# JiaoXianjun/multi-rtl-sdr-calibration

Hardware: AMD Instinct MI355X
Metric: IQ Msamples/s through FCCH+SCH calib (higher is better)
Workload: dtype f64; 1 GPU; cfg4 full chain gsm_sync_demod.m:107-124: 64 dongle streams (64/GPU) x 1020000 IQ samples (102 frames), fir1(46), FCCH+SCH+total_ppm_calculation, table on the host; streams_per_gpu=64, streams_total=64, output=table, collective=none, rows_checked_vs_oracle_per_rank=0

## Files before the change

### include/gsmcal.h

```cpp
#ifndef GSMCAL_H
#define GSMCAL_H

#include <stddef.h>
#include <stdint.h>

#ifdef __cplusplus
extern "C" {
#endif

typedef struct gsmcal_ctx gsmcal_ctx;

enum {
    GSMCAL_OK = 0,
    GSMCAL_S_NO_FCCH = 1,
    GSMCAL_S_FEW_HITS = 2,
    GSMCAL_S_FINE_FEW = 3,
    GSMCAL_S_FINE_SPACING = 4,
    GSMCAL_S_FINE_FEW_BURSTS = 5,
    GSMCAL_S_FINE_LOW_SNR = 6,
    GSMCAL_S_SCH_EDGE = 7,
    GSMCAL_S_SCH_FEW = 8,
    GSMCAL_S_SCH_SPACING = 9,
    GSMCAL_S_POST_NO_POS = 10,
    GSMCAL_S_POST_FEW_BCCH = 11,
// ... 247 lines not shown
int gsmcal_allgather_table(gsmcal_ctx* ctx, gsmcal_comm* comm, const double* d_local, int rows_per_rank, int cols,
                           double* d_all);

int gsmcal_allgather_table_async(gsmcal_ctx* ctx, gsmcal_comm* comm, const double* d_local, int rows_per_rank, int cols,
                                 double* d_all, int slot);
int gsmcal_allgather_wait(gsmcal_ctx* ctx, int slot);
int gsmcal_allgather_sync(gsmcal_ctx* ctx, int slot);

typedef struct gsmcal_ring gsmcal_ring;
int gsmcal_ring_create(gsmcal_ctx* ctx, size_t batch_bytes, int slots, gsmcal_ring** out);
void gsmcal_ring_destroy(gsmcal_ring* ring);
void* gsmcal_ring_host(gsmcal_ring* ring, int slot);
int gsmcal_ring_submit(gsmcal_ring* ring, int slot, size_t bytes);
void* gsmcal_ring_acquire(gsmcal_ring* ring, int slot);
int gsmcal_ring_release(gsmcal_ring* ring, int slot);
int gsmcal_ring_host_ready(gsmcal_ring* ring, int slot);

int gsmcal_synth_expand_dev(gsmcal_ctx* ctx, const uint8_t* d_base, int k, long n, uint8_t* d_out, long d,
                            long first_unit, unsigned long long seed);

int gsmcal_last_batch_details(gsmcal_ctx* ctx, int d, double* coarse_pos, double* coarse_snr,
                              double* fine_first, double* fcch_pos, double* sch_first, int* counts);

int gsmcal_last_batch_snr(gsmcal_ctx* ctx, int stream, double* snr, long cap, long* n_table, long* n_moving);

#ifdef __cplusplus
}
#endif
#endif
```

### multi-rtl-sdr-calibration_amd/__init__.py

```python
from . import build, ingest, synth
from ._lib import GsmcalError, MAX_HITS, MAX_POS_ROWS, MAX_SUBBANDS, TABLE_COLS, DEMOD_COLS, MAX_BCCH, BCCH_COLS, SCH_COLS, HYPERFRAME, CW_MAX_EVENTS, CW_COLS, CW_TILE, CW_OK, CW_SHORT, CW_ZERO, SIGNATURES, lib_path, load
from .api import (
    Context, default_context, raw2iq, filter, chn_filter_8x_4x, chn_filter_4x, move_fft_snr_runtime_avg,
    specific_fft_snr_fix_avg, FCCH_coarse_position, FCCH_fine_correction, SCH_corr_rate_correction,
    carrier_correct_post_SCH, total_ppm_calculation, SCH_equalise, frontend_batch, fcch_scan_batch, calibrate_batch,
    last_batch_details, last_batch_snr, TABLE_FIELDS, fcch_scan_batch_dev, calibrate_batch_dev, synth_expand_dev,
    set_verbose, last_call_report, num2str, band_power_batch, band_power_batch_dev, split_spectrum_scan,
    diversity_spectrum_scan, FCCH_demod, fcch_demod_batch, fcch_demod_batch_dev, demod_rows, DEMOD_FIELDS,
    subband_power_batch, subband_power_batch_dev, multichannel_spectrum_scan, CW_check, cw_check_batch, cw_check_batch_dev,
    cw_rows, CW_FIELDS, BCCH_demod, bcch_demod_batch, bcch_demod_batch_dev, bcch_rows, BCCH_FIELDS,
    SCH_decode, sch_decode_batch, sch_decode_batch_dev, sch_rows, SCH_FIELDS, sch_alignment,
)
```

### multi-rtl-sdr-calibration_amd/_lib.py

```python
from __future__ import annotations

import ctypes as C
import os

from . import build as _build

_LIB = None

c_double_p = C.POINTER(C.c_double)
c_int_p = C.POINTER(C.c_int)
c_long_p = C.POINTER(C.c_long)
c_u8_p = C.POINTER(C.c_uint8)

MAX_HITS = 24
MAX_POS_ROWS = 6 * MAX_HITS
TABLE_COLS = 10
MAX_SUBBANDS = 16
CW_MAX_EVENTS = 16
CW_COLS = 5 + 2 * CW_MAX_EVENTS
CW_TILE = 2048
CW_OK, CW_SHORT, CW_ZERO = 0, 1, 2
DEMOD_COLS = 4 + 3 * MAX_HITS
MAX_BCCH = 4 * MAX_HITS
BCCH_COLS = 6 + 4 * MAX_BCCH
# ... 95 lines not shown
    "gsmcal_comm_init_file": (C.c_int, [C.c_void_p, C.c_char_p, C.c_int, C.c_int, C.POINTER(C.c_void_p)]),
    "gsmcal_last_batch_snr": (C.c_int, [C.c_void_p, C.c_int, c_double_p, C.c_long, c_long_p, c_long_p]),
    "gsmcal_comm_init_file_nonce": (C.c_int, [C.c_void_p, C.c_char_p, C.c_ulonglong, C.c_int, C.c_int, C.POINTER(C.c_void_p)]),
    "gsmcal_comm_default_nonce": (C.c_ulonglong, []),
    "gsmcal_comm_id_file_exchange": (C.c_int, [C.c_char_p, C.c_ulonglong, C.c_int, C.c_int, C.c_void_p, C.c_double]),
    "gsmcal_comm_id_file_exchange_aged": (C.c_int, [C.c_char_p, C.c_ulonglong, C.c_int, C.c_int, C.c_void_p, C.c_double]),
    "gsmcal_comm_id_file_remove": (C.c_int, [C.c_char_p]),
    "gsmcal_comm_destroy": (None, [C.c_void_p]),
    "gsmcal_allgather_table": (C.c_int, [C.c_void_p, C.c_void_p, C.c_void_p, C.c_int, C.c_int, C.c_void_p]),
    "gsmcal_allgather_table_async": (C.c_int, [C.c_void_p, C.c_void_p, C.c_void_p, C.c_int, C.c_int, C.c_void_p, C.c_int]),
    "gsmcal_allgather_wait": (C.c_int, [C.c_void_p, C.c_int]),
    "gsmcal_allgather_sync": (C.c_int, [C.c_void_p, C.c_int]),
    "gsmcal_ring_create": (C.c_int, [C.c_void_p, C.c_size_t, C.c_int, C.POINTER(C.c_void_p)]),
    "gsmcal_ring_destroy": (None, [C.c_void_p]),
    "gsmcal_ring_host": (C.c_void_p, [C.c_void_p, C.c_int]),
    "gsmcal_ring_submit": (C.c_int, [C.c_void_p, C.c_int, C.c_size_t]),
    "gsmcal_ring_acquire": (C.c_void_p, [C.c_void_p, C.c_int]),
    "gsmcal_ring_release": (C.c_int, [C.c_void_p, C.c_int]),
    "gsmcal_ring_host_ready": (C.c_int, [C.c_void_p, C.c_int]),
    "gsmcal_synth_expand_dev": (C.c_int, [C.c_void_p, C.c_void_p, C.c_int, C.c_long, C.c_void_p, C.c_long, C.c_long,
                                          C.c_ulonglong]),
    "gsmcal_last_batch_details": (C.c_int, [C.c_void_p, C.c_int, c_double_p, c_double_p, c_double_p, c_double_p,
                                            c_double_p, c_int_p]),
}


class Params(C.Structure):
    _fields_ = [("coarse_th_db", C.c_double), ("coarse_mv_factor", C.c_int), ("coarse_max_offset", C.c_int),
                ("min_hits", C.c_int), ("fine_max_offset", C.c_int), ("fine_max_ppm", C.c_double),
                ("fine_gate_snr_db", C.c_double), ("fine_noise_bw_hz", C.c_double), ("sch_max_offset", C.c_int),
                ("sch_max_ppm", C.c_double), ("post_min_bcch", C.c_int), ("scan_min_hits", C.c_int),
                ("scan_spacing", C.c_double), ("scan_spacing_idle", C.c_double), ("scan_tol", C.c_double)]


SIGNATURES.update({
    "gsmcal_params_default": (None, [C.POINTER(Params)]),
    "gsmcal_set_params": (C.c_int, [C.c_void_p, C.POINTER(Params)]),
    "gsmcal_get_params": (C.c_int, [C.c_void_p, C.POINTER(Params)]),
})


class GsmcalError(RuntimeError):
    pass


def lib_path():
# ... 43 lines not shown
```

### multi-rtl-sdr-calibration_amd/api.py

```python
from __future__ import annotations

import ctypes as C
import math
import os

import numpy as np

from . import _lib
from ._lib import BCCH_COLS, SCH_COLS, CW_COLS, CW_MAX_EVENTS, DEMOD_COLS, MAX_BCCH, MAX_HITS, MAX_POS_ROWS, TABLE_COLS, GsmcalError

_CTX = {}


_VERBOSE = [os.environ.get("GSMCAL_VERBOSE") == "1"]


def set_verbose(on=True):
    _VERBOSE[0] = bool(on)


def last_call_report(ctx=None):
    ctx = ctx or default_context()
    n = ctx.lib.gsmcal_last_call_report(ctx.h, None, 0)
    if n <= 0:
# ... 775 lines not shown
    ctx = ctx or default_context()
    coef = np.ascontiguousarray(coef, dtype=np.float64)
    vp = lambda p: C.c_void_p(p) if p else None
    ctx.check(ctx.lib.gsmcal_fcch_scan_batch_dev(ctx.h, C.c_void_p(d_raw), int(d), int(n), _dp(coef), len(coef),
                                                 C.c_void_p(d_snr_numhit), vp(d_positions), vp(d_pos_snr), vp(d_counts)),
              "fcch_scan_batch_dev")


def synth_expand_dev(d_base, k, n, d_out, d, first_unit=0, seed=20260101, ctx=None):
    ctx = ctx or default_context()
    ctx.check(ctx.lib.gsmcal_synth_expand_dev(ctx.h, C.c_void_p(d_base), int(k), int(n), C.c_void_p(d_out), int(d),
                                              int(first_unit), int(seed)), "synth_expand_dev")


def last_batch_snr(stream, ctx=None):
    ctx = ctx or default_context()
    buf = np.zeros(1 << 16)
    n_tab, n_mov = C.c_long(0), C.c_long(0)
    ctx.check(ctx.lib.gsmcal_last_batch_snr(ctx.h, int(stream), _dp(buf), len(buf), C.byref(n_tab), C.byref(n_mov)),
              "last_batch_snr")
    return buf[: min(n_tab.value, len(buf))].copy(), int(n_mov.value)


def last_batch_details(d, ctx=None):
    ctx = ctx or default_context()
    arrs = [np.zeros((d, MAX_HITS)) for _ in range(5)]
    counts = np.zeros((d, 5), dtype=np.int32)
    ctx.check(ctx.lib.gsmcal_last_batch_details(ctx.h, d, *[_dp(a) for a in arrs],
                                                counts.ctypes.data_as(_lib.c_int_p)), "last_batch_details")
    names = ("coarse_pos", "coarse_snr", "fine_first", "fcch_pos", "sch_first")
    out = {k: a for k, a in zip(names, arrs)}
    out["counts"] = counts
    return out
```

### multi-rtl-sdr-calibration_amd/csrc/abi_calls.h

```cpp
#pragma once

const char* gsmcal_version(void) { return GSMCAL_VERSION; }

void gsmcal_params_default(gsmcal_params* p) {
    if (!p) return;
    p->coarse_th_db = 10.0; p->coarse_mv_factor = 10; p->coarse_max_offset = 5; p->min_hits = 5;
    p->fine_max_offset = 64; p->fine_max_ppm = 4000.0; p->fine_gate_snr_db = 5.0; p->fine_noise_bw_hz = 200e3;
    p->sch_max_offset = 8; p->sch_max_ppm = 400.0; p->post_min_bcch = 4;
    p->scan_min_hits = 3; p->scan_spacing = 12500.0; p->scan_spacing_idle = 12500.0 + 1250.0; p->scan_tol = 50.0;
}

int gsmcal_set_params(gsmcal_ctx* c, const gsmcal_params* p) {
    if (!c || !p) return GSMCAL_E_ARG;
    RET_IF(pipe_join(c));
    gsmcal_params d;
    gsmcal_params_default(&d);
    if (p->coarse_mv_factor != d.coarse_mv_factor || p->coarse_max_offset != d.coarse_max_offset ||
        p->fine_max_offset != d.fine_max_offset || p->fine_noise_bw_hz != d.fine_noise_bw_hz || p->sch_max_offset != d.sch_max_offset) {
        c->err = "gsmcal_set_params: a geometry field differs from its default";
        return GSMCAL_E_UNSUPPORTED;
    }
    if (p->min_hits < 2 || p->min_hits > GSMCAL_MAX_HITS || p->scan_min_hits < 1 || p->post_min_bcch < 0) {
        c->err = "gsmcal_set_params: min_hits outside 2..GSMCAL_MAX_HITS, scan_min_hits < 1 or post_min_bcch < 0";
        return GSMCAL_E_ARG;
// ... 54 lines not shown
    gsmcal_ctx* c = new gsmcal_ctx();
    gsmcal_params_default(&c->params);
    c->device = device_id;
    c->stream = (hipStream_t)hip_stream;
    c->own_stream = false;
    c->lanes[0].stream = c->stream;
    c->cur = &c->lanes[0];
    const char* e = getenv("GSMCAL_LANES");
    if (e && atoi(e) >= 1) c->n_lanes_cfg = atoi(e) > MAX_LANES ? MAX_LANES : atoi(e);
    { int ncu = 0; if (hipDeviceGetAttribute(&ncu, hipDeviceAttributeMultiprocessorCount, c->device) == hipSuccess && ncu > 0) c->n_cu = ncu; }
    { int lds = 0; if (hipDeviceGetAttribute(&lds, hipDeviceAttributeMaxSharedMemoryPerMultiprocessor, c->device) == hipSuccess && lds > 0) c->lds_per_cu = (size_t)lds; }
    if (const char* e2 = getenv("GSMCAL_SNR_INLINE_MIN")) c->snr_inline_min = atoi(e2);
    if (const char* e2 = getenv("GSMCAL_SNR_INLINE_KEEP")) c->snr_inline_keep = atoi(e2);
    if (const char* e2 = getenv("GSMCAL_FRONT_NT")) c->front_nt = atoi(e2);
    if (const char* e2 = getenv("GSMCAL_SCAN_SPLIT")) c->scan_split = atoi(e2);
    const char* sst = getenv("GSMCAL_SCAN_STAGES");
    if (sst && atoi(sst) >= 1) c->scan_stages = atoi(sst);
    const char* lm = getenv("GSMCAL_LANE_MIN");
    if (lm && atoi(lm) >= 1) c->lane_min = atoi(lm);
    const char* ce = getenv("GSMCAL_CERT");
    if (ce) c->certify = atoi(ce) != 0;
    const char* sfe = getenv("GSMCAL_SNR_FULL");
    if (sfe) c->snr_full = atoi(sfe) != 0;
    const char* sse = getenv("GSMCAL_SNR_SCREEN_DB");
    if (sse) c->snr_screen_db = atof(sse);
    const char* fge = getenv("GSMCAL_FUSE_GATHER");
    if (fge) c->fuse_fine_gather = atoi(fge) != 0;
    const char* fpe = getenv("GSMCAL_FUSE_POST");
    if (fpe) c->fuse_post = atoi(fpe) != 0;
    const char* pse = getenv("GSMCAL_POST_SLOTS");
    if (pse && atoi(pse) >= 1) c->post_slots_cap = atoi(pse);
    const char* pe = getenv("GSMCAL_PRESCREEN");
    if (pe && atoi(pe) == 0) c->prescreen = false;
    const char* fg = getenv("GSMCAL_FRONT_GENERIC");
    if (fg && atoi(fg) != 0) c->front_generic = true;
    if (const char* e2 = getenv("GSMCAL_FUSED_POLL_S")) { if (atof(e2) > 0.0) c->fused_poll_s = atof(e2); }
    if (const char* e2 = getenv("GSMCAL_TEST_FUSED_STALL")) c->test_stall = atoi(e2);
    const char* ge = getenv("GSMCAL_GRAPH");
    if (ge && atoi(ge) == 0) c->use_graph = false;
    if (ge && atoi(ge) == 2) c->graph_always = true;
    fused_gate_register(c);
    *out = c;
    return 0;
}

int gsmcal_ctx_create(int device_id, gsmcal_ctx** out) {
// ... 251 lines not shown
    if (!num || ntaps <= 0) { num = GSM_CHN_FILTER_4X_NUM; ntaps = 30; }
    return gsmcal_filter(c, num, ntaps, s, n, d, 1, r);
}

static int coarse_api(gsmcal_ctx* c, const double* s, long len, CoarseArgs a, StreamState* out) {
    ENTER(c);
    int fft_len = a.fft_len;
    long n_first = len;
    if (a.mode == 0) {
        fft_len = a.decimation_ratio > 74 ? 0 : 1 << (int)floor(log2(148.0 / (double)a.decimation_ratio));
        n_first = (long)ceil(23.0 * 1250.0 / (double)a.decimation_ratio);
    }
    if (fft_len < 2 || fft_len > 64) return GSMCAL_E_UNSUPPORTED;
    const long nwin = n_first - (fft_len - 1);
    const size_t lds = coarse_scan_lds(n_first > 0 ? n_first : 0, a.mode == 0 ? 10 * fft_len : a.mv_len);
    if (lds > 159 * 1024) return GSMCAL_E_UNSUPPORTED;
    RET_IF(upload_array(c, s, (size_t)len));
    std::vector<StreamState> v(1);
    host_init_state(v[0], len);
    RET_IF(push_states(c, v));
    c->last_S = 1; c->cur = &c->lanes[0]; c->lanes[0].lo = 0; c->lanes[0].n = 1; c->n_lanes_used = 1;
    a.s = (const cplx*)c->arr_in.p; a.s_stride = len; a.len = len;
    a.th0 = c->params.coarse_th_db; a.min_hits = c->params.min_hits;
    if (a.mode != 2 && nwin >= 1 && n_first <= len) {
        RET_IF(ensure(c, c->cur->snrbuf, (size_t)nwin * sizeof(double)));
        a.snr_g = (double*)c->cur->snrbuf.p; a.snr_stride = nwin;
        if (fft_len == 16) LAUNCH(c, k_coarse_snr<true>, dim3((unsigned)((nwin + 255) / 256), 1), dim3(256), 0, a);
        else LAUNCH(c, k_coarse_snr<false>, dim3((unsigned)((nwin + 255) / 256), 1), dim3(256), 0, a);
    }
    if (fft_len == 16) LAUNCH(c, k_coarse_scan_lat, dim3(1), dim3(256), lds, (StreamState*)c->cur->state.p, a);
    else LAUNCH(c, k_coarse_scan_gen, dim3(1), dim3(256), lds, (StreamState*)c->cur->state.p, a);
    CHECK_LAUNCH(c);
    RET_IF(fetch_states(c, 1, v));
    *out = v[0];
    return 0;
}

int gsmcal_move_fft_snr_runtime_avg(gsmcal_ctx* c, const double* s, long len, int mv_len, int fft_len, double th,
                                    int* hit_flag, double* hit_idx, double* hit_avg_snr, double* hit_snr) {
    if (!c || !s || len < 1 || mv_len < 1 || fft_len < 2) return GSMCAL_E_ARG;
    CoarseArgs a;
    memset(&a, 0, sizeof(a));
    a.mode = 1; a.mv_len = mv_len; a.fft_len = fft_len; a.th = th; a.decimation_ratio = 8;
    StreamState st;
    RET_IF(coarse_api(c, s, len, a, &st));
    if (st.status < 0) return st.status;
// ... 1020 lines not shown
```

### multi-rtl-sdr-calibration_amd/csrc/abi_util.h

```cpp
#pragma once
int gsmcal_synth_expand_dev(gsmcal_ctx* c, const uint8_t* d_base, int k, long n, uint8_t* d_out, long d, long first_unit,
                            unsigned long long seed) {
    if (!c || !d_base || !d_out || k < 1 || n < 1 || d < 1 || first_unit < 0) return GSMCAL_E_ARG;
    ENTER(c);
    c->cur = &c->lanes[0];
    for (long lo = 0; lo < d; lo += 32768) {
        const long cnt = d - lo < 32768 ? d - lo : 32768;
        long bx = (n / 8 + 255) / 256;
        if (bx > 64) bx = 64;
        LAUNCH(c, k_synth_expand, dim3((unsigned)bx, (unsigned)cnt), dim3(256), 0, d_base, k, n, d_out + (size_t)lo * 2 * n,
               first_unit + lo, seed);
    }
    CHECK_LAUNCH(c);
    return 0;
}

int gsmcal_last_batch_details(gsmcal_ctx* c, int d, double* coarse_pos, double* coarse_snr, double* fine_first,
                              double* fcch_pos, double* sch_first, int* counts) {
    if (!c || d < 1 || d > c->last_S) return GSMCAL_E_ARG;
    ENTER(c);
    HIPCHK(c, hipStreamSynchronize(c->stream));
    std::vector<StreamState> v((size_t)c->last_S);
    if (c->n_lanes_used <= 1 && c->lanes[0].n == 0) { c->lanes[0].lo = 0; c->lanes[0].n = c->last_S; }
    for (int i = 0; i < c->n_lanes_used; ++i) {
        const Lane& L = c->detail_lane ? *c->detail_lane : c->lanes[i];
        if (L.n <= 0 || L.lo + L.n > c->last_S) continue;
        HIPCHK(c, hipMemcpy(v.data() + L.lo, L.state.p, (size_t)L.n * sizeof(StreamState), hipMemcpyDeviceToHost));
    }
    for (int s = 0; s < d; ++s) {
        const StreamState& st = v[s];
        for (int i = 0; i < MAXH; ++i) {
            if (coarse_pos) coarse_pos[(size_t)s * MAXH + i] = i < st.n_coarse ? st.coarse_pos[i] : 0.0;
            if (coarse_snr) coarse_snr[(size_t)s * MAXH + i] = i < st.n_coarse ? st.coarse_snr[i] : 0.0;
            if (fine_first) fine_first[(size_t)s * MAXH + i] = i < st.n_fine ? st.fine_first[i] : 0.0;
            if (fcch_pos) fcch_pos[(size_t)s * MAXH + i] = i < st.n_fcch ? st.fcch_pos[i] : 0.0;
            if (sch_first) sch_first[(size_t)s * MAXH + i] = i < st.n_sch_first ? st.sch_first[i] : 0.0;
        }
        if (counts) {
            counts[5 * s + 0] = st.n_coarse;
            counts[5 * s + 1] = st.n_fine;
            counts[5 * s + 2] = st.fcch_is_sentinel ? -1 : st.n_fcch;
            counts[5 * s + 3] = st.n_sch_first;
            counts[5 * s + 4] = st.n_rows;
        }
    }
    return 0;
}

long gsmcal_coarse_scan_lds_fixed(void) { return (long)coarse_scan_lds_fixed(); }

int gsmcal_last_batch_snr(gsmcal_ctx* c, int stream, double* snr, long cap, long* n_table, long* n_moving) {
    if (!c || stream < 0 || stream >= c->last_S || !snr || cap < 1) return GSMCAL_E_ARG;
    ENTER(c);
    HIPCHK(c, hipStreamSynchronize(c->stream));
    for (int i = 0; i < c->n_lanes_used; ++i) {
        const Lane& L = c->detail_lane ? *c->detail_lane : c->lanes[i];
        if (stream < L.lo || stream >= L.lo + L.n) continue;
        if (L.snr_stride <= 0 && L.snr_nmove > 0) {
            c->err = "the last batch kept no SNR table (throughput batches compute the window SNRs inside the scan kernel; GSMCAL_SNR_INLINE_KEEP=1 writes it out)";
            return GSMCAL_E_UNSUPPORTED;
        }
        if (!L.snrbuf.p || L.snr_stride <= 0) continue;
        const long n = L.snr_stride < cap ? L.snr_stride : cap;
        HIPCHK(c, hipMemcpy(snr, (const double*)L.snrbuf.p + (size_t)(stream - L.lo) * L.snr_stride, (size_t)n * sizeof(double), hipMemcpyDeviceToHost));
        if (n_table) *n_table = L.snr_stride;
        if (n_moving) *n_moving = L.snr_nmove;
        return 0;
// ... 134 lines not shown
```

### multi-rtl-sdr-calibration_amd/csrc/host_plan.h

```cpp
#pragma once
namespace {

struct DevBuf {
    void* p = nullptr;
    size_t cap = 0;
};

struct ProfRec {
    int name_id;
    hipEvent_t e0, e1;
};

}

#define MAX_LANES 32
#define ALL_BUFS(Owner, ...)                                                                                                        \
    template <class F> void for_each_buf(F f) {                                                                                     \
        DevBuf* all[] = {__VA_ARGS__};                                                                                              \
        static_assert(sizeof(all) / sizeof(all[0]) == sizeof(Owner) / sizeof(DevBuf), #Owner ": a DevBuf is missing from for_each_buf"); \
        for (DevBuf* b : all) f(*b);                                                                                                \
    }
struct LaneBufs {
    DevBuf state, dec, win, peaks, snrbuf, x0, chunkrec, openlist, cert, partial, tailctr, xch, xepoch;
    ALL_BUFS(LaneBufs, &state, &dec, &win, &peaks, &snrbuf, &x0, &chunkrec, &openlist, &cert, &partial, &tailctr, &xch, &xepoch)
// ... 44 lines not shown
        unsigned long used = 0;
        int fused_streams = 0;
    };
    static constexpr int GRAPH_SLOTS = 4;
    GraphSlot g_calib[GRAPH_SLOTS], g_scan[GRAPH_SLOTS];
    unsigned long g_stamp = 0;
    unsigned long ws_epoch = 0;
    bool use_graph = true;
    bool graph_always = false;
    bool prescreen = true;
    int n_cu = 256;
    size_t lds_per_cu = 160 * 1024;
    int snr_inline_min = 1;
    int snr_inline_keep = 0;
    int front_nt = -1;
    size_t call_raw_bytes = 0;
    const void* last_raw = nullptr;
    bool call_raw_fresh = false;
    int scan_split = 88;
    int scan_stages = 0;
    int lane_min = 64;
    bool certify = true;
    bool snr_full = true;
    double snr_screen_db = 5.0;
    bool fuse_fine_gather = true;
    static constexpr int FUSED_MAX_STREAMS = 1024;
    std::vector<unsigned> fused_expected;
    unsigned* fused_done = nullptr;
    int fused_hi = 0;
    unsigned long long n_fused_launches = 0, n_gate_fallbacks = 0;
    int capture_fused_streams = 0;
    struct FusedCall {
        const uint8_t* d_raw; int d; long n; int ntaps, len_ts;
        std::vector<double> coef, ts, cf;
        double* d_table; double* d_pos_info; double* d_r_correct; long* d_r_len;
    };
    std::vector<FusedCall> fused_calls;
    double fused_poll_s = 3.0;
    int test_stall = 0;
    unsigned long long n_tail_reruns = 0;
    bool recovering = false;
    bool fuse_post = true;
    bool front_generic = false;
    bool capturing = false;
    static constexpr int PIPE_MAX_DEPTH = 8;
    int pipe_depth = 1;
// ... 743 lines not shown

int coarse(gsmcal_ctx* c, int S, const cplx* d_dec, long stride, long len, int dec_ratio, int fine_setup_ov,
           bool mean_corr = false, long n0 = 0, int front_decim = 64, const ScanAccept* accept = nullptr, bool allow_inline = true) {
    CoarseArgs a;
    memset(&a, 0, sizeof(a));
    if (accept) { a.accept = *accept; a.P = dev_params(c); }
    if (mean_corr) {
        a.mean_corr = 1;
        a.partial = (const unsigned long long*)c->cur->partial.p;
        a.npartial = c->cur->npartial;
        a.n0 = n0;
        double cs = 0.0;
        for (double v : c->h_coef) cs += v;
        a.csum_all = cs;
        const int ntaps = (int)c->h_coef.size();
        const int n_head = ntaps > 1 ? (ntaps - 1 + front_decim - 1) / front_decim : 1;
        if ((int)c->h_head.size() != n_head || c->head_epoch != c->coef_epoch) { c->err = "coarse(): csum_head not prepared"; return GSMCAL_E_ARG; }
        a.csum_head = (const double*)c->csum_head.p;
        a.n_head = n_head;
    }
    a.s = d_dec; a.s_stride = stride; a.len = len; a.decimation_ratio = dec_ratio; a.mode = 0;
    a.th0 = c->params.coarse_th_db; a.min_hits = c->params.min_hits;
    a.fine_setup_ov = fine_setup_ov;
    const int fft_len = 1 << (int)floor(log2(148.0 / (double)dec_ratio));
    const long n_first = (long)ceil(23.0 * 1250.0 / (double)dec_ratio);
    const long nwin = n_first - (fft_len - 1);
    a.g_fft_len = fft_len; a.g_n_first = n_first;
    const size_t lds = coarse_scan_lds(n_first, 10 * fft_len);
    if (lds > 159 * 1024 || nwin < 1) return GSMCAL_E_UNSUPPORTED;
    long ntab = nwin;
    unsigned sblocks = (unsigned)((nwin + 255) / 256);
    if (fft_len == 16 && 2 * S <= c->n_cu && c->snr_full && !c->no_fuse_now && len - (fft_len - 1) > nwin) {
        ntab = len - (fft_len - 1);
        a.snr_nwin = ntab;
        a.snr_screen_db = c->snr_screen_db;
        {
            const double rho = pow(10.0, a.snr_screen_db / 10.0);
            const double gx = (0.9238795325112867 * rho - 1.0) / (rho + 1.0);
            a.snr_gx2 = gx > 0.0 ? gx * gx * (1.0 - 1e-9) : 0.0;
        }
        const long rest = ntab - nwin;
        if ((rest + sblocks - 1) / sblocks > CS_TILE - 3) sblocks = (unsigned)((rest + CS_TILE - 4) / (CS_TILE - 3));
        a.snr_tile = (int)((((rest + sblocks - 1) / sblocks) + 3) & ~3L);
    }
    const bool refg = dec_ratio == 8 && fft_len == 16 && n_first == 3594;
    if (allow_inline && refg && a.snr_nwin == 0 && c->snr_inline_min > 0 && S >= c->snr_inline_min) {
// ... 318 lines not shown
```

### multi-rtl-sdr-calibration_amd/csrc/kernels_detect.h

```cpp
#pragma once
#include "state.h"
#include "kernels_frontend.h"

__device__ __forceinline__ constexpr int fft16_rev(int k) { return ((k & 1) << 3) | ((k & 2) << 1) | ((k & 4) >> 1) | ((k & 8) >> 3); }
__device__ __forceinline__ void fft16(cplx* x) {
    const double c1 = 0.92387953251128673848, s1 = 0.38268343236508978178;
    const double r2 = 0.70710678118654752440;
    const cplx w16[8] = {{1.0, 0.0}, {c1, -s1}, {r2, -r2}, {s1, -c1}, {0.0, -1.0}, {-s1, -c1}, {-r2, -r2}, {-c1, -s1}};
#pragma unroll
    for (int len = 16; len >= 2; len >>= 1) {
        const int half = len >> 1, step = 16 / len;
#pragma unroll
        for (int i = 0; i < 16; i += len) {
#pragma unroll
            for (int j = 0; j < half; ++j) {
                const cplx u = x[i + j], v = x[i + j + half];
                x[i + j] = make_double2(u.x + v.x, u.y + v.y);
                const cplx d = make_double2(u.x - v.x, u.y - v.y);
                const int t = j * step;
                if (t == 0) x[i + j + half] = d;
                else if (t == 4) x[i + j + half] = make_double2(d.y, -d.x);
                else x[i + j + half] = cmul(d, w16[t]);
            }
        }
    }
}

template <int L>
__device__ __forceinline__ double snr_from_power(const double (&P)[L], double floor2 = -1.0) {
    double pm = P[L - 1], pc = P[0], pp = P[1 % L];
#pragma unroll
    for (int k = 1; k < L; ++k) {
        const bool h = P[k] > pc;
        pm = h ? P[k - 1] : pm;
        pp = h ? P[(k + 1) % L] : pp;
        pc = h ? P[k] : pc;
    }
    double sig = pm + pc;
    sig = sig + pp;
    double tot = 0.0;
#pragma unroll
    for (int k = 0; k < L; ++k) tot += P[k];
    const double noise = tot - sig;
    if (tot <= floor2) return __longlong_as_double(0x7ff8000000000000LL);
    return 10.0 * log10(sig / noise);
}

struct DecView {
    const cplx* s;
    double cr, ci;
    double mr, mi;
    const double* head;
    int n_head;
    double floor2;
};
__device__ __forceinline__ cplx dv_fix(const DecView& v, cplx x, long j) {
    if (j < v.n_head) { const double h = v.head[j]; return make_double2(x.x - v.mr * h, x.y - v.mi * h); }
    return make_double2(x.x - v.cr, x.y - v.ci);
}
__device__ __forceinline__ cplx dv_load(const DecView& v, long j) {
    const cplx x = v.s[j];
    if (j < v.n_head) { const double h = v.head[j]; return make_double2(x.x - v.mr * h, x.y - v.mi * h); }
    return make_double2(x.x - v.cr, x.y - v.ci);
}

// ... 68 lines not shown
struct ScanAccept {
    double* snr_numhit; double* positions; double* pos_snr; int* counts;
};
struct CoarseArgs {
    const cplx* s; long s_stride; long len;
    int decimation_ratio;
    int mode;
    int mv_len, fft_len; double th;
    long t_lo, t_hi; double avg_snr;
    double* snr_g; long snr_stride;
    long snr_nwin;
    ScanAccept accept; DevParams P;
    double snr_screen_db;
    int snr_tile;
    int fine_setup_ov;
    double csum_all;
    const double* csum_head; int n_head;
    int mean_corr;
    double th0; int min_hits;
    const unsigned long long* partial;
    int npartial; long n0;
    double snr_gx2;
    int g_fft_len; long g_n_first;
};

__device__ __forceinline__ void stream_mean(const CoarseArgs& a, int stream, double* mr, double* mi,
                                            unsigned long long* tot_i, unsigned long long* tot_q) {
    __shared__ unsigned long long sh_tot[2];
    if (threadIdx.x < 64) {
        unsigned long long si = 0, sq = 0;
        const unsigned long long* p = a.partial + (size_t)stream * a.npartial * 2;
        for (int b = threadIdx.x; b < a.npartial; b += 64) { si += p[2 * b]; sq += p[2 * b + 1]; }
        for (int off = 32; off > 0; off >>= 1) {
            si += __shfl_down(si, off, 64);
            sq += __shfl_down(sq, off, 64);
        }
        if (threadIdx.x == 0) { sh_tot[0] = si; sh_tot[1] = sq; }
    }
    __syncthreads();
    *tot_i = sh_tot[0]; *tot_q = sh_tot[1];
    *mr = (double)sh_tot[0] / (double)a.n0;
    *mi = (double)sh_tot[1] / (double)a.n0;
}

__device__ __forceinline__ DecView dec_view(const CoarseArgs& a, int stream, double mean_re, double mean_im) {
    DecView v;
// ... 454 lines not shown
                if (!(fabs(v) <= cert_V) || !(fabs(mg) > cert_delta)) { atomicMin(&sh_unc, j); break; }
                if (mg > 0.0) { atomicMin(&sh_pred, j); break; }
                sm += v - snr_s[j];
            }
        }
        __syncthreads();
      }
        if (tid < 64) {
            const int pred = sh_pred;
            const bool ok = !(sh_unc < pred);
            double sm = 0.0;
            if (ok && pred != 0x7fffffff) {
                for (int q = tid; q < mv_len; q += 64) sm += snr_s[pred + q];
            }
            sm = wave_sum(sm);
            if (tid == 0) {
                if (!ok) sh_exact = 1;
                else if (pred != 0x7fffffff) { sh_hit = pred; sh_avg = sm / (double)mv_len; }
            }
        }
        __syncthreads();
    }
    CS_STAMP(2);
    if (!bad && a.mode != 2) {
      for (int pass = 0; pass < 2; ++pass) {
        const long nwin = g.nwin;
        const double dmv = (double)mv_len;
        const bool exact = sh_exact != 0;
        if (tid < 64 && exact) {
            const int lane = tid;
            double sum_snr = 0.0;
            for (int i = 0; i < mv_len; ++i) sum_snr += 999.0;
            for (int base = 0; base < (int)nwin; base += 64) {
                const int i = base + lane;
                const double nw = snr_s[mv_len + i];
                double mine = 0.0;
                const double* So = snr_s + base;
                const double* Sn = snr_s + mv_len + base;
#pragma unroll
                for (int j0 = 0; j0 < 64; j0 += 8) {
                    double o[8], v[8];
#pragma unroll
                    for (int u = 0; u < 8; ++u) {
                        v[u] = Sn[j0 + u];
                        o[u] = So[j0 + u];
                    }
// ... 66 lines not shown
                        int src;
                        long ncur;
                        if (h0) {
                            src = __ffs(h0) - 1;
                            ncur = nx0 - max_offset + src;
                        } else if (g1ok) {
                            if (u1 & (h1 ? (2u << (__ffs(h1) - 1)) - 1u : gmask)) { redo = true; break; }
                            if (!h1) break;
                            src = __ffs(h1) - 1;
                            ncur = nx1 - max_offset + src;
                            src += 16;
                        } else break;
                        if (lane == src) {
                            st->coarse_pos[nn] = (double)((ncur - 1) * dec + 1);
                            st->coarse_snr[nn] = v;
                        }
                        cur = ncur;
                        ++nn;
                    }
                    if (lane == 0) {
                        sh_n = nn;
                        if (redo) sh_redo = 1;
                        st->n_coarse = nn;
                    }
                }
                __syncthreads();
                n = sh_n;
            } else {
                if (tw_lazy) make_tw();
                __shared__ long sh_cur;
                __shared__ int sh_stop, sh_need1, sh_took1;
                const int lane = tid & 63;
                const double hit_avg_snr = st->hit_avg_snr;
                const int dec = a.decimation_ratio;
                const long d0 = (long)round(12500.0 / (double)dec);
                const long d1 = (long)round(13750.0 / (double)dec);
                const int max_offset = 5, nt = 2 * max_offset + 1;
                const long limit = (len - (fft_len - 1)) - max_offset;
                long cur = hit + 1;
                n = 1;
                if (tid == 0) {
                    st->coarse_pos[0] = (double)((cur - 1) * dec + 1);
                    st->coarse_snr[0] = st->mv_hit_snr;
                    sh_stop = 0; sh_need1 = 0; sh_took1 = 0;
                }
                const double R = exp10((hit_avg_snr + th) / 10.0);
                const double r_eps = 0.2303 * cert_delta + 1e-12;
                const double Rhi = R * (1.0 + r_eps), Rlo = R * (1.0 - r_eps);
                double* hop_sig = hop_sig_base;
                constexpr bool fast = FFT16;
                const bool ratio_mode = !exact && fast;
                cplx pf = make_double2(0.0, 0.0);
                long pg = -1;
                long pbase0 = 0, pbase1 = 0;
                bool have_pf = false;
                const cplx* sraw = s.s;
                const int dw = tid >> 4, dk = tid & 15;
                __syncthreads();
#ifdef GSMCAL_DEVTIMING
                unsigned long long cyc[5] = {0, 0, 0, 0, 0}, c0 = 0;
#define HOP_CYC(i) do { const unsigned long long c1 = __builtin_readcyclecounter(); cyc[i] += c1 - c0; c0 = c1; } while (0)
#else
#define HOP_CYC(i) do { } while (0)
#endif
                while (n < MAXH) {
                    const long nx0 = cur + d0, nx1 = cur + d1;
                    if (nx0 > limit) break;
#ifdef GSMCAL_DEVTIMING
                    c0 = __builtin_readcyclecounter();
#endif
                    const bool g1ok = nx1 <= limit;
                    const bool took1 = sh_took1 != 0;
                    int r0 = 0, r1 = 1, off0 = 0, off1 = 0;
                    if (fast) {
                        if (have_pf) {
                            if (tid < 4 * CS_ROW) rows[tid] = pg < 0 ? make_double2(0.0, 0.0) : dv_fix(s, pf, pg);
                            r0 = took1 ? 2 : 0; r1 = r0 + 1;
                            off0 = (int)((nx0 - 6) - ((took1 ? pbase1 : pbase0) + d0));
                            off1 = (int)((nx1 - 6) - ((took1 ? pbase1 : pbase0) + d1));
                        } else if (tid < 64) {
                            const int gq = tid >> 5, i = tid & 31;
                            if (i < 26) {
                                const long gi = (gq ? nx1 : nx0) - 6 + i;
                                rows[gq * CS_ROW + i] = (gi >= 0 && gi < len && (gq == 0 || g1ok)) ? dv_load(s, gi) : make_double2(0.0, 0.0);
                            }
                        }
                        if (tid < 4 * CS_ROW) {
                            const int rr = tid / CS_ROW, i = tid - rr * CS_ROW;
// ... 93 lines not shown
                                        else st->coarse_snr[n] = v;
                                        sh_cur = ncur; sh_took1 = grp; sh_need1 = 0;
                                    }
                                } else if (grp == 0 && g1ok) {
                                    if (lane == 0) sh_need1 = 1;
                                } else if (lane == 0) sh_stop = 1;
                            }
                        }
                        HOP_CYC(3);
                        __syncthreads();
                        if (sh_stop || !sh_need1) break;
                    }
                    if (sh_stop) break;
                    cur = sh_cur;
                    ++n;
                    __syncthreads();
                    HOP_CYC(4);
                }
#ifdef GSMCAL_DEVTIMING
                if (g_stamps && tid == 0 && blockIdx.x < DEV_STAMP_BLOCKS) {
                    unsigned long long* r = g_stamps + ((size_t)KID_COARSE_SCAN * DEV_STAMP_BLOCKS + blockIdx.x) * 16;
                    unsigned long long acc = r[0];
                    r[8] = acc;
                    for (int i = 0; i < 5; ++i) { acc += cyc[i]; r[9 + i] = acc; }
                    r[14] = acc + 100ull * (unsigned long long)n;
                }
#endif
                __syncthreads();
                if (ratio_mode && tid >= 1 && tid < n)
                    st->coarse_snr[tid] = 10.0 * log10(hop_sig[2 * tid] / hop_sig[2 * tid + 1]);
                if (tid == 0) st->n_coarse = n;
            }
        }
        __syncthreads();
        const int redo = sh_redo;
        __syncthreads();
        if (!redo) break;
        if (tid == 0) {
            sh_exact = 1; sh_redo = 0; sh_hit = 0x7fffffff;
            st->n_coarse = 0; st->coarse_hit_flag = 0; st->hit_avg_snr = INFINITY; st->mv_hit_idx = -1.0; st->mv_hit_snr = INFINITY;
        }
        n = 0;
        __syncthreads();
      }
      CS_STAMP(4);
    } else if (!bad) {
        const long lo = a.t_lo, hi = a.t_hi;
        if (hi >= lo) {
            if (lo < 1) {
                if (tid == 0) set_status(st, 3, GSMCAL_E_INDEX);
            } else {
                const long hi_fit = hi + fft_len - 1 > len ? len - (fft_len - 1) : hi;
                const long cnt = hi_fit >= lo ? hi_fit - lo + 1 : 0;
                for (long i = tid; i < cnt; i += 256) snr_s[i] = FFT16 ? window_snr16(s, lo - 1 + i) : window_snr_generic(s, lo - 1 + i, fft_len, tw);
                __syncthreads();
                if (tid == 0) {
                    bool hit = false;
                    for (long i = 0; i < cnt && !hit; ++i)
                        if (snr_s[i] - a.avg_snr > th) {
                            st->coarse_hit_flag = 1;
                            st->mv_hit_idx = (double)(lo + i);
                            st->mv_hit_snr = snr_s[i];
                            hit = true;
// ... 1071 lines not shown
```

### multi-rtl-sdr-calibration_amd/csrc/state.h

```cpp
#pragma once
#include <hip/hip_runtime.h>
#include <stdint.h>
#include "../../include/gsmcal.h"

#ifdef GSMCAL_DEVTIMING
__device__ unsigned long long* g_stamps = nullptr;
#define DEV_STAMP_BLOCKS 1024
#ifdef GSMCAL_DEVTIMING_LIGHT
#ifndef GSMCAL_DEVTIMING_MASK
#define GSMCAL_DEVTIMING_MASK 0x601
#endif
#define DEV_STAMP_ON(kid, i) ((kid) == GSMCAL_DEVTIMING_LIGHT && ((GSMCAL_DEVTIMING_MASK >> (i)) & 1))
#else
#define DEV_STAMP_ON(kid, i) true
#endif
#define DEV_STAMP(kid, blk, i)                                                                          \
    do {                                                                                                \
        if (DEV_STAMP_ON(kid, i) && g_stamps && threadIdx.x == 0 && (blk) < DEV_STAMP_BLOCKS)          \
            g_stamps[((size_t)(kid) * DEV_STAMP_BLOCKS + (blk)) * 16 + (i)] = wall_clock64();          \
    } while (0)
#else
#define DEV_STAMP(kid, blk, i) do { } while (0)
#endif
enum { KID_COARSE_SNR = 0, KID_COARSE_SCAN, KID_GATHER, KID_CERT, KID_CHUNK, KID_VERIFY, KID_BT1, KID_SCH, KID_BT0, KID_FRONT, KID_N };
// ... 4 lines not shown
enum { OP_NONE = 0, OP_LERP = 1, OP_MIX = 2, OP_COPY = 3 };
enum { SRC_ARR = 0, SRC_RAW = 1 };
#define NLEVELS 5

struct LevelOp {
    int type;
    int pad;
    double param;
    long n;
};

struct alignas(16) StreamState {
    long n0;
    unsigned long long sum_i, sum_q;
    double mean_re, mean_im;
    LevelOp op[NLEVELS];
    int n_coarse;
    int coarse_hit_flag;
    double coarse_pos[MAXH];
    double coarse_snr[MAXH];
    double hit_avg_snr;
    double mv_hit_idx, mv_hit_snr;
    int n_win;
    long win_start[MAXH];
    int n_fine_ws;
    long fine_ws[MAXH];
    int n_fine;
    double fine_first[MAXH];
    int n_fcch;
    int fcch_is_sentinel;
    double fcch_pos[MAXH];
    double sampling_ppm1, carrier_ppm1;
    double fo_burst[MAXH], snr_burst[MAXH];
    int prior_bin[MAXH];
    int r1_kind;
    int n_sch_first;
    int sch_edge;
    double sch_first[MAXH];
    int n_sch;
    double sch_pos[MAXH];
    double sampling_ppm2;
    int r2_kind;
    int n_rows;
    int n_sent_rows;
    double pos_info[2 * MAXROWS];
    double carrier_ppm2;
    int r3_kind;
    int status;
// ... 19 lines not shown
```

Before: 548,200 Msample/s.

## Precompute FCCH hop hit map in parallel to replace serial coarse hop loop

Before the serial coarse FCCH hop search, each wavefront computes 16-point FFT SNR decisions for candidate windows around the predicted next-hop positions. It stores hit, uncertain and usable bitmasks in shared memory. The hop walk then resolves up to twelve hops from these masks and recomputes exact per-hop power in two parallel passes, falling back to the original loop on ambiguity. This targets the latency of the sequential per-hop FFT and barrier chain, at the cost of speculative FFT work, extra shared memory reuse and added per-stream state fields.

After: 550,100 Msample/s (median of 3 runs). No clear change (+0.3%).

```diff
diff --git a/include/gsmcal.h b/include/gsmcal.h
--- a/include/gsmcal.h
+++ b/include/gsmcal.h
@@ -293,6 +293,8 @@
 int gsmcal_last_batch_details(gsmcal_ctx* ctx, int d, double* coarse_pos, double* coarse_snr,
                               double* fine_first, double* fcch_pos, double* sch_first, int* counts);
 
+int gsmcal_last_batch_hop_route(gsmcal_ctx* ctx, int d, int* map_hops, int* loop_hops);
+
 int gsmcal_last_batch_snr(gsmcal_ctx* ctx, int stream, double* snr, long cap, long* n_table, long* n_moving);
 
 #ifdef __cplusplus
diff --git a/multi-rtl-sdr-calibration_amd/__init__.py b/multi-rtl-sdr-calibration_amd/__init__.py
--- a/multi-rtl-sdr-calibration_amd/__init__.py
+++ b/multi-rtl-sdr-calibration_amd/__init__.py
@@ -4,7 +4,7 @@
     Context, default_context, raw2iq, filter, chn_filter_8x_4x, chn_filter_4x, move_fft_snr_runtime_avg,
     specific_fft_snr_fix_avg, FCCH_coarse_position, FCCH_fine_correction, SCH_corr_rate_correction,
     carrier_correct_post_SCH, total_ppm_calculation, SCH_equalise, frontend_batch, fcch_scan_batch, calibrate_batch,
-    last_batch_details, last_batch_snr, TABLE_FIELDS, fcch_scan_batch_dev, calibrate_batch_dev, synth_expand_dev,
+    last_batch_details, last_batch_snr, last_batch_hop_route, TABLE_FIELDS, fcch_scan_batch_dev, calibrate_batch_dev, synth_expand_dev,
     set_verbose, last_call_report, num2str, band_power_batch, band_power_batch_dev, split_spectrum_scan,
     diversity_spectrum_scan, FCCH_demod, fcch_demod_batch, fcch_demod_batch_dev, demod_rows, DEMOD_FIELDS,
     subband_power_batch, subband_power_batch_dev, multichannel_spectrum_scan, CW_check, cw_check_batch, cw_check_batch_dev,
diff --git a/multi-rtl-sdr-calibration_amd/_lib.py b/multi-rtl-sdr-calibration_amd/_lib.py
--- a/multi-rtl-sdr-calibration_amd/_lib.py
+++ b/multi-rtl-sdr-calibration_amd/_lib.py
@@ -141,6 +141,7 @@
                                           C.c_ulonglong]),
     "gsmcal_last_batch_details": (C.c_int, [C.c_void_p, C.c_int, c_double_p, c_double_p, c_double_p, c_double_p,
                                             c_double_p, c_int_p]),
+    "gsmcal_last_batch_hop_route": (C.c_int, [C.c_void_p, C.c_int, c_int_p, c_int_p]),
 }
 
 
diff --git a/multi-rtl-sdr-calibration_amd/api.py b/multi-rtl-sdr-calibration_amd/api.py
--- a/multi-rtl-sdr-calibration_amd/api.py
+++ b/multi-rtl-sdr-calibration_amd/api.py
@@ -821,6 +821,14 @@
     return buf[: min(n_tab.value, len(buf))].copy(), int(n_mov.value)
 
 
+def last_batch_hop_route(d, ctx=None):
+    ctx = ctx or default_context()
+    mh, lh = np.zeros(d, dtype=np.int32), np.zeros(d, dtype=np.int32)
+    ctx.check(ctx.lib.gsmcal_last_batch_hop_route(ctx.h, int(d), mh.ctypes.data_as(_lib.c_int_p), lh.ctypes.data_as(_lib.c_int_p)),
+              "last_batch_hop_route")
+    return mh, lh
+
+
 def last_batch_details(d, ctx=None):
     ctx = ctx or default_context()
     arrs = [np.zeros((d, MAX_HITS)) for _ in range(5)]
diff --git a/multi-rtl-sdr-calibration_amd/csrc/abi_calls.h b/multi-rtl-sdr-calibration_amd/csrc/abi_calls.h
--- a/multi-rtl-sdr-calibration_amd/csrc/abi_calls.h
+++ b/multi-rtl-sdr-calibration_amd/csrc/abi_calls.h
@@ -100,6 +100,8 @@
     if (ce) c->certify = atoi(ce) != 0;
     const char* sfe = getenv("GSMCAL_SNR_FULL");
     if (sfe) c->snr_full = atoi(sfe) != 0;
+    const char* hme = getenv("GSMCAL_HOP_MAP");
+    if (hme) c->hop_map = atoi(hme) != 0;
     const char* sse = getenv("GSMCAL_SNR_SCREEN_DB");
     if (sse) c->snr_screen_db = atof(sse);
     const char* fge = getenv("GSMCAL_FUSE_GATHER");
@@ -397,6 +399,7 @@
     c->last_S = 1; c->cur = &c->lanes[0]; c->lanes[0].lo = 0; c->lanes[0].n = 1; c->n_lanes_used = 1;
     a.s = (const cplx*)c->arr_in.p; a.s_stride = len; a.len = len;
     a.th0 = c->params.coarse_th_db; a.min_hits = c->params.min_hits;
+    a.hop_map = c->hop_map ? 1 : 0;
     if (a.mode != 2 && nwin >= 1 && n_first <= len) {
         RET_IF(ensure(c, c->cur->snrbuf, (size_t)nwin * sizeof(double)));
         a.snr_g = (double*)c->cur->snrbuf.p; a.snr_stride = nwin;
diff --git a/multi-rtl-sdr-calibration_amd/csrc/abi_util.h b/multi-rtl-sdr-calibration_amd/csrc/abi_util.h
--- a/multi-rtl-sdr-calibration_amd/csrc/abi_util.h
+++ b/multi-rtl-sdr-calibration_amd/csrc/abi_util.h
@@ -43,6 +43,24 @@
             counts[5 * s + 3] = st.n_sch_first;
             counts[5 * s + 4] = st.n_rows;
         }
+    }
+    return 0;
+}
+
+int gsmcal_last_batch_hop_route(gsmcal_ctx* c, int d, int* map_hops, int* loop_hops) {
+    if (!c || d < 1 || d > c->last_S) return GSMCAL_E_ARG;
+    ENTER(c);
+    HIPCHK(c, hipStreamSynchronize(c->stream));
+    std::vector<StreamState> v((size_t)c->last_S);
+    if (c->n_lanes_used <= 1 && c->lanes[0].n == 0) { c->lanes[0].lo = 0; c->lanes[0].n = c->last_S; }
+    for (int i = 0; i < c->n_lanes_used; ++i) {
+        const Lane& L = c->detail_lane ? *c->detail_lane : c->lanes[i];
+        if (L.n <= 0 || L.lo + L.n > c->last_S) continue;
+        HIPCHK(c, hipMemcpy(v.data() + L.lo, L.state.p, (size_t)L.n * sizeof(StreamState), hipMemcpyDeviceToHost));
+    }
+    for (int s = 0; s < d; ++s) {
+        if (map_hops) map_hops[s] = v[s].hops_map;
+        if (loop_hops) loop_hops[s] = v[s].hops_loop;
     }
     return 0;
 }
diff --git a/multi-rtl-sdr-calibration_amd/csrc/host_plan.h b/multi-rtl-sdr-calibration_amd/csrc/host_plan.h
--- a/multi-rtl-sdr-calibration_amd/csrc/host_plan.h
+++ b/multi-rtl-sdr-calibration_amd/csrc/host_plan.h
@@ -90,6 +90,7 @@
     int lane_min = 64;
     bool certify = true;
     bool snr_full = true;
+    bool hop_map = true;
     double snr_screen_db = 5.0;
     bool fuse_fine_gather = true;
     static constexpr int FUSED_MAX_STREAMS = 1024;
@@ -879,6 +880,7 @@
     a.s = d_dec; a.s_stride = stride; a.len = len; a.decimation_ratio = dec_ratio; a.mode = 0;
     a.th0 = c->params.coarse_th_db; a.min_hits = c->params.min_hits;
     a.fine_setup_ov = fine_setup_ov;
+    a.hop_map = c->hop_map ? 1 : 0;
     const int fft_len = 1 << (int)floor(log2(148.0 / (double)dec_ratio));
     const long n_first = (long)ceil(23.0 * 1250.0 / (double)dec_ratio);
     const long nwin = n_first - (fft_len - 1);
diff --git a/multi-rtl-sdr-calibration_amd/csrc/kernels_detect.h b/multi-rtl-sdr-calibration_amd/csrc/kernels_detect.h
--- a/multi-rtl-sdr-calibration_amd/csrc/kernels_detect.h
+++ b/multi-rtl-sdr-calibration_amd/csrc/kernels_detect.h
@@ -26,8 +26,38 @@
     }
 }
 
+__device__ __forceinline__ cplx fft16_stage1(cplx u, cplx v, int i, int hf) {
+    const double c1 = 0.92387953251128673848, s1 = 0.38268343236508978178, r2 = 0.70710678118654752440;
+    const cplx w16[8] = {{1.0, 0.0}, {c1, -s1}, {r2, -r2}, {s1, -c1}, {0.0, -1.0}, {-s1, -c1}, {-r2, -r2}, {-c1, -s1}};
+    if (hf == 0) return make_double2(u.x + v.x, u.y + v.y);
+    const cplx d = make_double2(u.x - v.x, u.y - v.y);
+    if (i == 0) return d;
+    if (i == 4) return make_double2(d.y, -d.x);
+    return cmul(d, w16[i]);
+}
+__device__ __forceinline__ void fft16_half(cplx* x) {
+    const double r2 = 0.70710678118654752440;
+#pragma unroll
+    for (int len = 8; len >= 2; len >>= 1) {
+        const int half = len >> 1, step = 16 / len;
+#pragma unroll
+        for (int i = 0; i < 8; i += len) {
+#pragma unroll
+            for (int j = 0; j < half; ++j) {
+                const cplx u = x[i + j], v = x[i + j + half];
+                x[i + j] = make_double2(u.x + v.x, u.y + v.y);
+                const cplx d = make_double2(u.x - v.x, u.y - v.y);
+                const int t = j * step;
+                if (t == 0) x[i + j + half] = d;
+                else if (t == 4) x[i + j + half] = make_double2(d.y, -d.x);
+                else x[i + j + half] = cmul(d, t == 2 ? make_double2(r2, -r2) : make_double2(-r2, -r2));
+            }
+        }
+    }
+}
+
 template <int L>
-__device__ __forceinline__ double snr_from_power(const double (&P)[L], double floor2 = -1.0) {
+__device__ __forceinline__ void sig_tot_from_power(const double (&P)[L], double* sig_out, double* tot_out, double* peak_out) {
     double pm = P[L - 1], pc = P[0], pp = P[1 % L];
 #pragma unroll
     for (int k = 1; k < L; ++k) {
@@ -41,6 +71,12 @@
     double tot = 0.0;
 #pragma unroll
     for (int k = 0; k < L; ++k) tot += P[k];
+    *sig_out = sig; *tot_out = tot; *peak_out = pc;
+}
+template <int L>
+__device__ __forceinline__ double snr_from_power(const double (&P)[L], double floor2 = -1.0) {
+    double sig, tot, pc;
+    sig_tot_from_power<L>(P, &sig, &tot, &pc);
     const double noise = tot - sig;
     if (tot <= floor2) return __longlong_as_double(0x7ff8000000000000LL);
     return 10.0 * log10(sig / noise);
@@ -155,6 +191,7 @@
     int npartial; long n0;
     double snr_gx2;
     int g_fft_len; long g_n_first;
+    int hop_map;
 };
 
 __device__ __forceinline__ void stream_mean(const CoarseArgs& a, int stream, double* mr, double* mi,
@@ -655,6 +692,111 @@
         __syncthreads();
     }
     CS_STAMP(2);
+    constexpr int HM_K = 12, HM_W = 49, HM_LEFT = 28, HM_PER_WAVE = HM_K / 2, HM_RC = 12;
+    static_assert(HM_W + 15 <= 64, "a cluster's samples are one load per lane");
+    static_assert(4 * 64 * sizeof(cplx) <= 4 * CS_ROW * sizeof(cplx) + 2 * 11 * 17 * sizeof(double), "cluster staging fits rows | Pb");
+    static_assert(2 * HM_K * 3 * sizeof(unsigned long long) <= 48 * sizeof(cplx), "map words fit behind the 16 twiddles");
+    static_assert(HM_K < MAXH && MAXH <= 2 * HM_RC + 1, "two recompute passes cover every hop");
+    static_assert(HM_RC * (16 * sizeof(cplx) + 17 * sizeof(double)) <= 4 * CS_ROW * sizeof(cplx) + 2 * 11 * 17 * sizeof(double), "a recompute pass fits rows | Pb");
+    bool map_built = false;
+#ifdef GSMCAL_DEVTIMING
+    unsigned long long hm_cyc[3] = {0, 0, 0};
+#endif
+    if constexpr (FFT16) {
+        if (want_cert && a.hop_map && sh_exact == 0 && sh_hit != 0x7fffffff) {
+            unsigned long long* hm_words = (unsigned long long*)(tw + 16);
+#ifdef GSMCAL_DEVTIMING
+            const unsigned long long hm_c0 = __builtin_readcyclecounter();
+#endif
+            const int lane = tid & 63;
+            const double h_snr = snr_s[mv_len + sh_hit];
+            const double h_pta = h_snr - sh_avg;
+            const double hit_avg_snr = h_snr - h_pta;
+            const double R = exp10((hit_avg_snr + th) / 10.0);
+            const double r_eps = 0.2303 * cert_delta + 1e-12;
+            const double Rhi = R * (1.0 + r_eps), Rlo = R * (1.0 - r_eps);
+            const double tol_u = (1.0 + R) * 1.1102230246251565e-16;
+            const long d0 = (long)round(12500.0 / (double)a.decimation_ratio);
+            const long d1 = (long)round(13750.0 / (double)a.decimation_ratio);
+            const long cur = (long)sh_hit + 1;
+            const cplx* sraw = s.s;
+            const int wave_u = __builtin_amdgcn_readfirstlane(tid >> 6);
+            const int which = wave_u & 1;
+            cplx* xs = rows + wave_u * 64;
+            const int l0 = lane < HM_W ? lane : HM_W - 1;
+            const long last_w = len - 15;
+            auto slot_first = [&](int j) {
+                const int k = (wave_u >> 1) + 2 * j + 1, b = (k - 1 + 5 * which) / 5;
+                return cur + (long)(k - b) * d0 + (long)b * d1 - HM_LEFT;
+            };
+            auto slot_on = [&](long F) { return F <= last_w && F + (HM_W - 1) >= 1; };
+            auto slot_load = [&](int j) {
+                const long F = slot_first(j), gi = F - 1 + lane;
+                return (j < HM_PER_WAVE && slot_on(F) && gi >= 0 && gi < len) ? sraw[gi] : make_double2(0.0, 0.0);
+            };
+            cplx xnext = slot_load(0);
+#pragma unroll 1
+            for (int j = 0; j < HM_PER_WAVE; ++j) {
+                const cplx xc = xnext;
+                xnext = slot_load(j + 1);
+                const long F = slot_first(j);
+                unsigned long long* wd = hm_words + 3 * (2 * ((wave_u >> 1) + 2 * j) + which);
+                if (!slot_on(F)) {
+                    if (lane == 0) { wd[0] = 0ull; wd[1] = 0ull; wd[2] = 0ull; }
+                    continue;
+                }
+                __builtin_amdgcn_wave_barrier();
+                xs[lane] = xc;
+                double P[16];
+                double p0_raw = 0.0;
+#pragma unroll
+                for (int hf = 0; hf < 2; ++hf) {
+                    __builtin_amdgcn_fence(__ATOMIC_RELEASE, "wavefront");
+                    __builtin_amdgcn_wave_barrier();
+                    __builtin_amdgcn_fence(__ATOMIC_ACQUIRE, "wavefront");
+                    cplx y[8];
+#pragma unroll
+                    for (int i = 0; i < 8; ++i) {
+                        const cplx u = xs[l0 + i], v = xs[l0 + i + 8];
+                        y[i] = fft16_stage1(u, v, i, hf);
+                    }
+                    fft16_half(y);
+                    if (hf == 0) {
+                        p0_raw = y[0].x * y[0].x + y[0].y * y[0].y;
+                        y[0].x -= 16.0 * s.cr; y[0].y -= 16.0 * s.ci;
+                    }
+#pragma unroll
+                    for (int r = 0; r < 8; ++r) P[fft16_rev(8 * hf + r)] = y[r].x * y[r].x + y[r].y * y[r].y;
+                }
+                double m_sig, m_tot, m_pc;
+                sig_tot_from_power<16>(P, &m_sig, &m_tot, &m_pc);
+                double p_top = P[0] > P[1] ? P[0] : P[1], p_2nd = P[0] > P[1] ? P[1] : P[0];
+#pragma unroll
+                for (int q = 2; q < 16; ++q) {
+                    const double lo = P[q] < p_top ? P[q] : p_top;
+                    p_2nd = lo > p_2nd ? lo : p_2nd;
+                    p_top = P[q] > p_top ? P[q] : p_top;
+                }
+                const double m_noise = m_tot - m_sig;
+                const double tot_raw = (m_tot - P[0]) + p0_raw;
+                const double sq = sqrt(m_tot * tot_raw);
+                const bool alone = p_2nd < m_pc - 1.1102230246251565e-16 * (128.0 * sq + 4e-12 * tot_raw);
+                const long w = F + lane;
+                const bool usable = lane < HM_W && w >= 1 && w <= last_w && w - 1 >= (long)s.n_head && tot_raw < INFINITY &&
+                                    m_tot > 1e-24 * tot_raw && m_tot > 4.0 * s.floor2 && alone;
+                const double tol = tol_u * (330.0 * sq + 32.0 * m_tot + 2e-12 * tot_raw);
+                const bool okn = m_noise > 0.0 && m_noise < INFINITY && m_sig < INFINITY;
+                const bool m_hit = usable && okn && m_sig - tol > Rhi * m_noise;
+                const bool m_miss = usable && okn && m_sig + tol < Rlo * m_noise;
+                const unsigned long long hw = __ballot(m_hit), uw = __ballot(usable && !(m_hit || m_miss)), vw = __ballot(usable);
+                if (lane == 0) { wd[0] = hw; wd[1] = uw; wd[2] = vw; }
+            }
+#ifdef GSMCAL_DEVTIMING
+            hm_cyc[0] = __builtin_readcyclecounter() - hm_c0;
+#endif
+            map_built = true;
+        }
+    }
     if (!bad && a.mode != 2) {
       for (int pass = 0; pass < 2; ++pass) {
         const long nwin = g.nwin;
@@ -767,6 +909,7 @@
                         sh_n = nn;
                         if (redo) sh_redo = 1;
                         st->n_coarse = nn;
+                        st->hops_map = 0; st->hops_loop = nn - 1;
                     }
                 }
                 __syncthreads();
@@ -808,7 +951,106 @@
 #else
 #define HOP_CYC(i) do { } while (0)
 #endif
-                while (n < MAXH) {
+                bool map_final = false;
+                int map_hops = 0;
+                if constexpr (FFT16) {
+                  if (ratio_mode && map_built) {
+                    const unsigned long long* hm_words = (const unsigned long long*)(tw + 16);
+#ifdef GSMCAL_DEVTIMING
+                    unsigned long long hm_c0 = __builtin_readcyclecounter();
+#endif
+                    long my_w0 = 0, my_w1 = 0;
+                    {
+                        int b = 0;
+                        auto look = [&](int k, long nx, int bb, unsigned& h) {
+                            const int which = bb == (k - 1) / 5 ? 0 : (bb == (k + 4) / 5 ? 1 : -1);
+                            if (which < 0) return false;
+                            const long o = (nx - max_offset) - (cur + (long)(k - bb) * d0 + (long)bb * d1 - HM_LEFT);
+                            if (o < 0 || o + (nt - 1) > HM_W - 1) return false;
+                            const unsigned long long* wd = hm_words + 3 * (2 * (k - 1) + which);
+                            const unsigned gm = (1u << nt) - 1u;
+                            h = (unsigned)(wd[0] >> o) & gm;
+                            const unsigned un = (unsigned)(wd[1] >> o) & gm, us = (unsigned)(wd[2] >> o) & gm;
+                            const unsigned looked = h ? (2u << (__ffs(h) - 1)) - 1u : gm;
+                            return ((un | ~us) & looked) == 0u;
+                        };
+                        long wcur = cur;
+                        int wn = n;
+                        while (wn < MAXH && wn <= HM_K) {
+                            const long nx0 = wcur + d0, nx1 = wcur + d1;
+                            if (nx0 > limit) { map_final = true; break; }
+                            unsigned h = 0;
+                            if (!look(wn, nx0, b, h)) break;
+                            long ncur;
+                            if (h) ncur = nx0 - max_offset + (__ffs(h) - 1);
+                            else if (nx1 <= limit) {
+                                if (!look(wn, nx1, b + 1, h)) break;
+                                if (!h) { map_final = true; break; }
+                                ncur = nx1 - max_offset + (__ffs(h) - 1);
+                                ++b;
+                            } else { map_final = true; break; }
+                            if (tid == 0) st->coarse_pos[wn] = (double)((ncur - 1) * dec + 1);
+                            if (wn == 1 + dw) my_w0 = ncur;
+                            if (wn == 1 + HM_RC + dw) my_w1 = ncur;
+                            wcur = ncur;
+                            ++wn;
+                        }
+                        map_hops = wn - n;
+                        cur = wcur;
+                        n = wn;
+                    }
+#ifdef GSMCAL_DEVTIMING
+                    { const unsigned long long c1 = __builtin_readcyclecounter(); hm_cyc[1] = c1 - hm_c0; hm_c0 = c1; }
+#endif
+                    for (int pass = 0; pass < 2 && map_hops > 0 && HM_RC * pass + 1 < n; ++pass) {
+                        cplx* hx = rows;
+                        double* hp = (double*)(rows + HM_RC * 16);
+                        const int hi = HM_RC * pass + 1 + dw;
+                        const bool on = dw < HM_RC && hi < n;
+                        if (on) hx[tid] = dv_load(s, (pass ? my_w1 : my_w0) - 1 + dk);
+                        __syncthreads();
+                        if (on) {
+                            const cplx* x = hx + dw * 16;
+                            double pr_[4] = {0.0, 0.0, 0.0, 0.0}, pi_[4] = {0.0, 0.0, 0.0, 0.0};
+#pragma unroll
+                            for (int m = 0; m < 16; ++m) {
+                                const cplx t = tw[(dk * m) & 15], xv = x[m];
+                                pr_[m & 3] = fma(xv.x, t.x, pr_[m & 3]); pi_[m & 3] = fma(xv.x, t.y, pi_[m & 3]);
+                                pr_[m & 3] = fma(-xv.y, t.y, pr_[m & 3]); pi_[m & 3] = fma(xv.y, t.x, pi_[m & 3]);
+                            }
+                            const double xr = (pr_[0] + pr_[1]) + (pr_[2] + pr_[3]), xi = (pi_[0] + pi_[1]) + (pi_[2] + pi_[3]);
+                            hp[dw * 17 + dk] = fma(xi, xi, xr * xr);
+                        }
+                        __syncthreads();
+                        if (on && dk == 0) {
+                            double P[16];
+                            const double* pr = hp + dw * 17;
+#pragma unroll
+                            for (int k = 0; k < 16; ++k) P[k] = pr[k];
+                            double mv[8]; int mi[8];
+#pragma unroll
+                            for (int k = 0; k < 8; ++k) { const bool r = P[2 * k + 1] > P[2 * k]; mv[k] = r ? P[2 * k + 1] : P[2 * k]; mi[k] = 2 * k + (r ? 1 : 0); }
+#pragma unroll
+                            for (int w = 4; w >= 1; w >>= 1)
+#pragma unroll
+                                for (int k = 0; k < w; ++k) { const bool r = mv[2 * k + 1] > mv[2 * k]; mv[k] = r ? mv[2 * k + 1] : mv[2 * k]; mi[k] = r ? mi[2 * k + 1] : mi[2 * k]; }
+                            const double pc = mv[0], pm = pr[(mi[0] + 15) & 15], pp = pr[(mi[0] + 1) & 15];
+                            double sig = pm + pc;
+                            sig = sig + pp;
+                            double t8[8];
+#pragma unroll
+                            for (int k = 0; k < 8; ++k) t8[k] = P[2 * k] + P[2 * k + 1];
+                            const double tot = ((t8[0] + t8[1]) + (t8[2] + t8[3])) + ((t8[4] + t8[5]) + (t8[6] + t8[7]));
+                            hop_sig[2 * hi] = sig; hop_sig[2 * hi + 1] = tot - sig;
+                        }
+                        __syncthreads();
+                    }
+#ifdef GSMCAL_DEVTIMING
+                    { const unsigned long long c1 = __builtin_readcyclecounter(); hm_cyc[2] = c1 - hm_c0; }
+#endif
+                  }
+                }
+                while (n < MAXH && !map_final) {
                     const long nx0 = cur + d0, nx1 = cur + d1;
                     if (nx0 > limit) break;
 #ifdef GSMCAL_DEVTIMING
@@ -948,14 +1190,22 @@
                     unsigned long long* r = g_stamps + ((size_t)KID_COARSE_SCAN * DEV_STAMP_BLOCKS + blockIdx.x) * 16;
                     unsigned long long acc = r[0];
                     r[8] = acc;
-                    for (int i = 0; i < 5; ++i) { acc += cyc[i]; r[9 + i] = acc; }
-                    r[14] = acc + 100ull * (unsigned long long)n;
+                    if (hm_cyc[0]) {
+                        for (int i = 0; i < 3; ++i) { acc += hm_cyc[i]; r[9 + i] = acc; }
+                        for (int i = 0; i < 5; ++i) acc += cyc[i];
+                        r[12] = acc;
+                        acc += 100ull * (unsigned long long)map_hops; r[13] = acc;
+                        r[14] = acc + 100ull * (unsigned long long)(n - 1 - map_hops);
+                    } else {
+                        for (int i = 0; i < 5; ++i) { acc += cyc[i]; r[9 + i] = acc; }
+                        r[14] = acc + 100ull * (unsigned long long)n;
+                    }
                 }
 #endif
                 __syncthreads();
                 if (ratio_mode && tid >= 1 && tid < n)
                     st->coarse_snr[tid] = 10.0 * log10(hop_sig[2 * tid] / hop_sig[2 * tid + 1]);
-                if (tid == 0) st->n_coarse = n;
+                if (tid == 0) { st->n_coarse = n; st->hops_map = map_hops; st->hops_loop = n - 1 - map_hops; }
             }
         }
         __syncthreads();
@@ -965,6 +1215,7 @@
         if (tid == 0) {
             sh_exact = 1; sh_redo = 0; sh_hit = 0x7fffffff;
             st->n_coarse = 0; st->coarse_hit_flag = 0; st->hit_avg_snr = INFINITY; st->mv_hit_idx = -1.0; st->mv_hit_snr = INFINITY;
+            st->hops_map = 0; st->hops_loop = 0;
         }
         n = 0;
         __syncthreads();
diff --git a/multi-rtl-sdr-calibration_amd/csrc/state.h b/multi-rtl-sdr-calibration_amd/csrc/state.h
--- a/multi-rtl-sdr-calibration_amd/csrc/state.h
+++ b/multi-rtl-sdr-calibration_amd/csrc/state.h
@@ -50,8 +50,10 @@
     double hit_avg_snr;
     double mv_hit_idx, mv_hit_snr;
     int n_win;
+    int hops_map;
     long win_start[MAXH];
     int n_fine_ws;
+    int hops_loop;
     long fine_ws[MAXH];
     int n_fine;
     double fine_first[MAXH];
```
